# LIS-TU-Berlin/SVN-ICP

Measured on AMD Instinct MI355X. Metric: scan-pair registrations/sec at N particles x M source pts, 1/2/4/8 GPU, higher is better.
Workload: dtype f64; 1 GPU; C3: 128 particles SVN-ICP, 131072-pt source vs 262144-pt target, K=100, I=20, max_dist=1.0, lr=1.0, SVNFullGrad=False, correspondence=fast, early stop off; synthetic 64-beam scans (seed 20250718); particles=128, target_points=262144, knn_count=100, parallelism=single GPU

## Files before the change

### svn-icp_amd/csrc/knn_tiles.hip

```cpp
#include "kernels.hpp"
#include "stein_split_device.hpp"

namespace svnicp {

namespace {

constexpr int T = 8;
constexpr int STEP = kWave * T;
constexpr int QW = 64;
constexpr int WAVES = 4;
constexpr int QCAP = 1024;
constexpr int SL = 512;
constexpr int NSQ = 4;
constexpr int MAX_TILES = 8192;
constexpr int QB = 16;
constexpr double kU = 5.9604644775390625e-08;
constexpr float kEpsTile = 56.0f * 5.9604644775390625e-08f;

struct alignas(16) QF { float x, y, z, thr; };
struct alignas(16) QD { double x, y, z, tau; };

__device__ __forceinline__ void wave_sync() {
  __builtin_amdgcn_fence(__ATOMIC_ACQ_REL, "wavefront");
  __builtin_amdgcn_wave_barrier();
}
__device__ __forceinline__ bool ent_less(double da, int ia, double db, int ib) {
  return (da < db) || (da == db && ia < ib);
}
__device__ void bitonic_sort(double* sd, int* si, int S, int lane) {
  for (int k = 2; k <= S; k <<= 1)
    for (int j = k >> 1; j > 0; j >>= 1) {
      for (int e = lane; e < (S >> 1); e += kWave) {
        const int a = ((e & ~(j - 1)) << 1) | (e & (j - 1)), b = a | j;
        const bool up = (a & k) == 0;
        const double da = sd[a], db = sd[b];
        const int ia = si[a], ib = si[b];
        if (ent_less(db, ib, da, ia) == up) { sd[a] = db; si[a] = ib; sd[b] = da; si[b] = ia; }
      }
      wave_sync();
    }
}
__device__ void bitonic_sort128_f32(float* v, int lane) {
  for (int k = 2; k <= 128; k <<= 1)
    for (int j = k >> 1; j > 0; j >>= 1) {
      const int a = ((lane & ~(j - 1)) << 1) | (lane & (j - 1)), b = a | j;
      const bool up = (a & k) == 0;
      const float va = v[a], vb = v[b];
      if ((vb < va) == up) { v[a] = vb; v[b] = va; }
      wave_sync();
    }
}
__device__ __forceinline__ float next_down(float f) {
  if (f == 0.0f) return -1.401298464e-45f;
  int b = __float_as_int(f); b += (f > 0.0f) ? -1 : 1; return __int_as_float(b);
}
__device__ __forceinline__ float next_up(float f) {
  if (f == 0.0f) return 1.401298464e-45f;
  int b = __float_as_int(f); b += (f > 0.0f) ? 1 : -1; return __int_as_float(b);
}
__device__ __forceinline__ float f32_floor(double v) { float f = (float)v; return ((double)f > v) ? next_down(f) : f; }
__device__ __forceinline__ float f32_ceil(double v) { float f = (float)v; return ((double)f < v) ? next_up(f) : f; }
__device__ __forceinline__ float f32_round_up(double v) {
  float f = (float)v;
  if ((double)f < v) f = __int_as_float(__float_as_int(f) + 1);
  return f;
}
__device__ __forceinline__ float filter_threshold(double tau, double E) {
  if (!(tau < __builtin_huge_val())) return __builtin_huge_valf();
  const double r = sqrt(tau) * (1.0 + 1e-15) + 3.4641016151377553 * kU * E;
  return f32_round_up((r * r) * (1.0 + 5.0 * kU + 1e-6));
}
__device__ __forceinline__ float box_lb2(float alo0, float alo1, float alo2, float ahi0, float ahi1, float ahi2,
                                         float blo0, float blo1, float blo2, float bhi0, float bhi1, float bhi2) {
  const float g0 = __builtin_fmaxf(0.0f, __builtin_fmaxf(blo0 - ahi0, alo0 - bhi0));
  const float g1 = __builtin_fmaxf(0.0f, __builtin_fmaxf(blo1 - ahi1, alo1 - bhi1));
  const float g2 = __builtin_fmaxf(0.0f, __builtin_fmaxf(blo2 - ahi2, alo2 - bhi2));
  return (g0 * g0 + g1 * g1 + g2 * g2) * 0.999999f;
}

struct alignas(16) QRec { double x, y, z, tau; int cnt; int row; float thr, tb; };

__device__ __forceinline__ int pool_read(const KnnTilesArgs& a, int64_t r, int e) {
  if (e < kTilesBase) return a.pool[r * kTilesBase + e];
  const int o = e - kTilesBase;
  const int id = a.chunk_tab[r * kTilesChunks + (o / kTilesChunk)];
  return a.arena[(int64_t)id * kTilesChunk + (o % kTilesChunk)];
}

struct P3 { double x, y, z; };
__device__ __forceinline__ P3 target_row(const KnnTilesArgs& a, bool on, int i) {
  P3 c{0.0, 0.0, 0.0};
  if (on) { const double* p = a.tgt + 3 * (int64_t)i; c.x = p[0]; c.y = p[1]; c.z = p[2]; }
  return c;
}
__device__ __forceinline__ void write_table_row(const KnnTilesArgs& a, int64_t b, int r0, const P3 c0, int r1, const P3 c1, double* sd, int lane) {
  const int K = a.K;
  const bool on0 = r0 >= 0 && r0 < K, on1 = r1 >= 0 && r1 < K;
  const double x0 = c0.x, y0 = c0.y, z0 = c0.z, x1 = c1.x, y1 = c1.y, z1 = c1.z;
  float* rb = reinterpret_cast<float*>(sd);
  double* anc = sd + 256;
  wave_sync();
  if (on0 && r0 == 0) { anc[0] = x0; anc[1] = y0; anc[2] = z0; }
  if (on1 && r1 == 0) { anc[0] = x1; anc[1] = y1; anc[2] = z1; }
  wave_sync();
  const double a0 = anc[0], a1 = anc[1], a2 = anc[2];
  if (on0) *reinterpret_cast<float4*>(rb + 4 * r0) = table_row(x0, y0, z0, a0, a1, a2);
  if (on1) *reinterpret_cast<float4*>(rb + 4 * r1) = table_row(x1, y1, z1, a0, a1, a2);
  for (int k = K + lane; k < 128; k += kWave) *reinterpret_cast<float4*>(rb + 4 * k) = table_sentinel_row();
  wave_sync();
  float cm = 0.0f;
  for (int k = lane; k < K; k += kWave) cm = table_row_cmax(cm, *reinterpret_cast<const float4*>(rb + 4 * k));
  cm = table_cmax_wave(cm);
  if (lane == 0) {
    a.tbl_cmax[b] = cm;
    a.tbl_anchor[3 * b] = a0; a.tbl_anchor[3 * b + 1] = a1; a.tbl_anchor[3 * b + 2] = a2;
  }
  table_store_rows(rb, a.tbl_a, b, lane);
}

__device__ void select_query(const KnnTilesArgs& a, int64_t r, const QRec& rec, double* sd, int* si, int lane) {
  const int K = a.K, S2 = a.S2;
  const int64_t b = rec.row;
  const int n_first = rec.cnt;
  const double qx = rec.x, qy = rec.y, qz = rec.z;
  double tau = rec.tau;
  if (a.stat_n && lane == 0) a.stat_n[b] = n_first;
  const int n = n_first;
  bool ok = n <= S2;
  int m = 0;
  constexpr int NBR = 8;
  static_assert(NBR * kWave == kTilesBase, "the register path reads the query's own pool row only");
  if (ok && n <= NBR * kWave) {
    int slot[NBR], orig[NBR];
    double d[NBR];
#pragma unroll
    for (int j = 0; j < NBR; ++j) {
      const int e = j * kWave + lane;
      slot[j] = (j * kWave < n && e < n) ? a.pool[r * (int64_t)kTilesBase + e] : -1;
    }
#pragma unroll
    for (int j = 0; j < NBR; ++j) {
      d[j] = __builtin_huge_val(); orig[j] = 0;
      if (j * kWave < n && slot[j] >= 0) {
        orig[j] = a.torig[slot[j]];
        const double dx = qx - a.tx[slot[j]], dy = qy - a.ty[slot[j]], dz = qz - a.tz[slot[j]];
        d[j] = (dx * dx + dy * dy) + dz * dz;
      }
    }
    if (n > 2 * kWave && n >= K) {
      auto count_le = [&](double t) -> int {
        int c = 0;
#pragma unroll
        for (int j = 0; j < NBR; ++j)
          if (j * kWave < n) c += __popcll(__ballot(slot[j] >= 0 && d[j] <= t));
        return c;
      };
      double lo = 0.0, hi = tau;
      if (!(hi < __builtin_huge_val())) {
        double mx = 0.0;
#pragma unroll
        for (int j = 0; j < NBR; ++j) if (slot[j] >= 0) mx = fmax(mx, d[j]);
        for (int off = 32; off > 0; off >>= 1) mx = fmax(mx, __shfl_xor(mx, off, kWave));
        hi = mx;
      }
      const double target = 0.5 * (K + 2 * kWave);
      double t = hi * (double)__builtin_powf((float)(target / n), 0.6666667f);
      for (int it = 0; it < 48; ++it) {
        if (!(t > lo && t < hi)) t = 0.5 * (lo + hi);
        if (!(t > lo && t < hi)) break;
        const int c = count_le(t);
        if (c < K) lo = t;
        else { hi = t; if (c <= 2 * kWave) break; }
        t = 0.5 * (lo + hi);
      }
      tau = hi < tau ? hi : tau;
    }
#pragma unroll
    for (int j = 0; j < NBR; ++j) {
      if (j * kWave < n) {
        const bool pass = slot[j] >= 0 && d[j] <= tau;
        const unsigned long long pm = __ballot(pass);
        const int pos = m + (int)__builtin_amdgcn_mbcnt_hi((unsigned int)(pm >> 32), __builtin_amdgcn_mbcnt_lo((unsigned int)pm, 0u));
        if (pass && pos < SL) { sd[pos] = d[j]; si[pos] = orig[j]; }
        m += __popcll(pm);
      }
    }
    ok = m >= K && m <= SL;
  } else if (ok) {
    if (n > SL / 2) {
      double m1 = __builtin_huge_val(), m2 = __builtin_huge_val();
      for (int e = lane; e < n; e += kWave) {
        const int slot = pool_read(a, r, e);
        const double dx = qx - a.tx[slot], dy = qy - a.ty[slot], dz = qz - a.tz[slot];
        const double d = (dx * dx + dy * dy) + dz * dz;
        m2 = d < m1 ? m1 : (d < m2 ? d : m2);
        m1 = d < m1 ? d : m1;
      }
      sd[2 * lane] = m1; sd[2 * lane + 1] = m2; si[2 * lane] = 0; si[2 * lane + 1] = 0;
      wave_sync();
      bitonic_sort(sd, si, 128, lane);
      const double t2 = sd[K - 1];
      wave_sync();
      tau = t2 < tau ? t2 : tau;
    }
    for (int e0 = 0; e0 < n; e0 += kWave) {
      const int e = e0 + lane;
      bool pass = false;
      double d = 0.0;
      int orig = 0;
      if (e < n) {
        const int slot = pool_read(a, r, e);
        orig = a.torig[slot];
        const double dx = qx - a.tx[slot], dy = qy - a.ty[slot], dz = qz - a.tz[slot];
        d = (dx * dx + dy * dy) + dz * dz;
        pass = d <= tau;
      }
      const unsigned long long pm = __ballot(pass);
      const int pos = m + (int)__builtin_amdgcn_mbcnt_hi((unsigned int)(pm >> 32), __builtin_amdgcn_mbcnt_lo((unsigned int)pm, 0u));
      if (pass && pos < SL) { sd[pos] = d; si[pos] = orig; }
      m += __popcll(pm);
    }
    ok = m >= K && m <= SL;
  }
  if (!ok) {
    if (lane == 0) {
      const int slot = atomicAdd(a.fail_count, 1);
      a.fail_list[slot] = (int32_t)b;
      if (a.fail_tau) a.fail_tau[slot] = (n <= S2 && m < K) ? __builtin_huge_val() : tau;
    }
    wave_sync();
    return;
  }
  if (m <= 2 * kWave) {
    for (int e = m + lane; e < 2 * kWave + 8; e += kWave) { sd[e] = __builtin_huge_val(); si[e] = 0x7fffffff; }
    wave_sync();
    const int e0 = lane, e1 = lane + kWave;
    const double d0 = e0 < m ? sd[e0] : 0.0, d1 = e1 < m ? sd[e1] : 0.0;
    const int i0 = e0 < m ? si[e0] : 0, i1 = e1 < m ? si[e1] : 0;
    const P3 c0 = target_row(a, a.tbl_a && e0 < m, i0), c1 = target_row(a, a.tbl_a && e1 < m, i1);
    int* flag = si + 2 * kWave + 8;
    flag[lane] = 0; flag[lane + kWave] = 0;
    int r0 = 0, r1 = 0;
    for (int j0 = 0; j0 < m; j0 += 8) {
      double dj[8];
#pragma unroll
      for (int u = 0; u < 8; ++u) dj[u] = sd[j0 + u];
#pragma unroll
      for (int u = 0; u < 8; ++u) {
        r0 += dj[u] < d0 ? 1 : 0;
        r1 += dj[u] < d1 ? 1 : 0;
      }
    }
    wave_sync();
    if (e0 < m) atomicAdd(&flag[r0], 1);
    if (e1 < m) atomicAdd(&flag[r1], 1);
    wave_sync();
    if (__ballot((e0 < m && flag[r0] > 1) || (e1 < m && flag[r1] > 1))) {
      for (int j = 0; j < m; ++j) {
        const double dj = sd[j];
        const int ij = si[j];
        r0 += (dj == d0 && ij < i0) ? 1 : 0;
        r1 += (dj == d1 && ij < i1) ? 1 : 0;
      }
    }
    if (e0 < m && r0 < K) { a.out_idx[b * K + r0] = i0; if (a.out_d2) a.out_d2[b * K + r0] = d0; }
    if (e1 < m && r1 < K) { a.out_idx[b * K + r1] = i1; if (a.out_d2) a.out_d2[b * K + r1] = d1; }
    if (a.tbl_a) write_table_row(a, b, e0 < m ? r0 : -1, c0, e1 < m ? r1 : -1, c1, sd, lane);
    wave_sync();
  } else {
    int S = 256;
    while (S < m) S <<= 1;
    for (int e = m + lane; e < S; e += kWave) { sd[e] = __builtin_huge_val(); si[e] = 0x7fffffff; }
    wave_sync();
    bitonic_sort(sd, si, S, lane);
    for (int e = lane; e < K; e += kWave) { a.out_idx[b * K + e] = si[e]; if (a.out_d2) a.out_d2[b * K + e] = sd[e]; }
    if (a.tbl_a) {
      const int e1 = lane + kWave;
      write_table_row(a, b, lane, target_row(a, lane < K, si[lane]), e1, target_row(a, e1 < K, e1 < K ? si[e1] : 0), sd, lane);
    }
    wave_sync();
  }
}

__global__ __launch_bounds__(256) void k_knn_seed(KnnTilesArgs a) {
  extern __shared__ __align__(16) unsigned char smem[];
  const int lane = threadIdx.x & (kWave - 1);
  const int wave = __builtin_amdgcn_readfirstlane(threadIdx.x >> 6);
  const int K = a.K, n_tiles = a.n_tiles;
  constexpr size_t kShared = sizeof(QD) * QW + sizeof(QF) * QW + 4 * sizeof(int) * QW + sizeof(unsigned int) * (MAX_TILES / 32);
  constexpr size_t kScratch = sizeof(float2) * QB * kWave + 512;
  static_assert(QB * WAVES == QW, "one batch per wave");
  QD* qd = reinterpret_cast<QD*>(smem);
  QF* qf = reinterpret_cast<QF*>(smem + sizeof(QD) * QW);
  int* cnt = reinterpret_cast<int*>(smem + (sizeof(QD) + sizeof(QF)) * QW);
  int* qb = cnt + QW;
  float* thrb = reinterpret_cast<float*>(qb + QW);
  int* spare = reinterpret_cast<int*>(thrb + QW);
  unsigned int* tbits = reinterpret_cast<unsigned int*>(spare + QW);
  unsigned char* scratch = smem + kShared + kScratch * wave;
  float2* lm = reinterpret_cast<float2*>(scratch);

  const unsigned int grp = blockIdx.x;
  const int64_t q0 = a.b_lo + (int64_t)grp * QW;
  const int nq = (a.b_hi - q0) < QW ? (int)(a.b_hi - q0) : QW;
  const double Et = __longlong_as_double((long long)*a.emax_bits);

  unsigned long long tphase = a.phase_cycles ? __builtin_readcyclecounter() : 0ull;
  unsigned long long pacc[8] = {0, 0, 0, 0, 0, 0, 0, 0};
  auto phase_mark = [&](int i) {
    if (!a.phase_cycles) return;
    const unsigned long long now = __builtin_readcyclecounter();
    pacc[i] += now - tphase;
    tphase = now;
  };
  float wlo0 = 0.f, wlo1 = 0.f, wlo2 = 0.f, whi0 = 0.f, whi1 = 0.f, whi2 = 0.f;
  const int nwords = (n_tiles + 31) >> 5;
  if (wave == 0) {
    const bool act = lane < nq;
    const int64_t b = act ? (int64_t)a.qorder[q0 - a.b_lo + lane] : 0;
    QD s; s.x = s.y = s.z = 0.0; s.tau = 0.0;
    if (act) {
      stage_a_query(a.pose, a.src[3 * b], a.src[3 * b + 1], a.src[3 * b + 2], &s.x, &s.y, &s.z);
    }
    qd[lane] = s;
    QF f; f.x = (float)s.x; f.y = (float)s.y; f.z = (float)s.z; f.thr = -1.0f;
    qf[lane] = f;
    cnt[lane] = 0; qb[lane] = (int)b; thrb[lane] = -1.0f;
    const float inf = __builtin_huge_valf();
    wlo0 = act ? f32_floor(s.x) : inf; wlo1 = act ? f32_floor(s.y) : inf; wlo2 = act ? f32_floor(s.z) : inf;
    whi0 = act ? f32_ceil(s.x) : -inf; whi1 = act ? f32_ceil(s.y) : -inf; whi2 = act ? f32_ceil(s.z) : -inf;
    for (int off = 32; off > 0; off >>= 1) {
      wlo0 = __builtin_fminf(wlo0, __shfl_xor(wlo0, off, kWave)); whi0 = __builtin_fmaxf(whi0, __shfl_xor(whi0, off, kWave));
      wlo1 = __builtin_fminf(wlo1, __shfl_xor(wlo1, off, kWave)); whi1 = __builtin_fmaxf(whi1, __shfl_xor(whi1, off, kWave));
      wlo2 = __builtin_fminf(wlo2, __shfl_xor(wlo2, off, kWave)); whi2 = __builtin_fmaxf(whi2, __shfl_xor(whi2, off, kWave));
    }
  }
  wave_sync();
  const float* bx_lo0 = a.tile_box, *bx_lo1 = a.tile_box + n_tiles, *bx_lo2 = a.tile_box + 2 * (size_t)n_tiles;
  const float* bx_hi0 = a.tile_box + 3 * (size_t)n_tiles, *bx_hi1 = a.tile_box + 4 * (size_t)n_tiles,
             * bx_hi2 = a.tile_box + 5 * (size_t)n_tiles;

  {
    if (wave == 0) {
      for (int e = lane; e < nwords; e += kWave) tbits[e] = 0u;
      wave_sync();
      const float px = qf[lane].x, py = qf[lane].y, pz = qf[lane].z;
      unsigned long long best[NSQ];
#pragma unroll
      for (int i = 0; i < NSQ; ++i) best[i] = ~0ull;
      float4* boxs = reinterpret_cast<float4*>(scratch);
      const int n_groups = (n_tiles + kWave - 1) / kWave;
      unsigned int gkey[2] = {0xffffffffu, 0xffffffffu};
      for (int g = 0; g < n_groups; ++g) {
        const int tl = g * kWave + lane;
        const float inf = __builtin_huge_valf();
        float lo0 = inf, lo1 = inf, lo2 = inf, hi0 = -inf, hi1 = -inf, hi2 = -inf;
        if (tl < n_tiles) { lo0 = bx_lo0[tl]; lo1 = bx_lo1[tl]; lo2 = bx_lo2[tl]; hi0 = bx_hi0[tl]; hi1 = bx_hi1[tl]; hi2 = bx_hi2[tl]; }
        for (int off = 32; off > 0; off >>= 1) {
          lo0 = __builtin_fminf(lo0, __shfl_xor(lo0, off, kWave)); hi0 = __builtin_fmaxf(hi0, __shfl_xor(hi0, off, kWave));
          lo1 = __builtin_fminf(lo1, __shfl_xor(lo1, off, kWave)); hi1 = __builtin_fmaxf(hi1, __shfl_xor(hi1, off, kWave));
          lo2 = __builtin_fminf(lo2, __shfl_xor(lo2, off, kWave)); hi2 = __builtin_fmaxf(hi2, __shfl_xor(hi2, off, kWave));
        }
        const float glb = box_lb2(wlo0, wlo1, wlo2, whi0, whi1, whi2, lo0, lo1, lo2, hi0, hi1, hi2);
        const unsigned int key = (glb < inf) ? ((__float_as_uint(glb) & ~127u) | (unsigned int)g) : 0xffffffffu;
        if (lane == (g & (kWave - 1))) gkey[g >> 6] = key;
      }
      for (;;) {
        unsigned int kmin = gkey[0] < gkey[1] ? gkey[0] : gkey[1];
        for (int off = 32; off > 0; off >>= 1) { const unsigned int o = __shfl_xor(kmin, off, kWave); kmin = o < kmin ? o : kmin; }
        if (kmin == 0xffffffffu) break;
        float w4 = -__builtin_huge_valf();
        if (lane < nq) w4 = best[NSQ - 1] == ~0ull ? __builtin_huge_valf() : __uint_as_float((unsigned int)(best[NSQ - 1] >> 32));
        for (int off = 32; off > 0; off >>= 1) w4 = __builtin_fmaxf(w4, __shfl_xor(w4, off, kWave));
        if (__uint_as_float(kmin & ~127u) > w4) break;
        const int gsel = (int)(kmin & 127u);
        if (lane == (gsel & (kWave - 1))) gkey[gsel >> 6] = 0xffffffffu;
        const int t0 = gsel * kWave;
        const int tl = t0 + lane;
        if (tl < n_tiles) {
          boxs[2 * lane] = make_float4(bx_lo0[tl], bx_lo1[tl], bx_lo2[tl], bx_hi0[tl]);
          boxs[2 * lane + 1] = make_float4(bx_hi1[tl], bx_hi2[tl], 0.f, 0.f);
        }
        wave_sync();
        const int cntt = (n_tiles - t0) < kWave ? (n_tiles - t0) : kWave;
#pragma unroll 4
        for (int i = 0; i < cntt; ++i) {
          const float4 b0 = boxs[2 * i], b1 = boxs[2 * i + 1];
          const float l0 = b0.x, l1 = b0.y, l2 = b0.z, h0 = b0.w, h1 = b1.x, h2 = b1.y;
          const int tile = t0 + i;
          const float lb = box_lb2(px, py, pz, px, py, pz, l0, l1, l2, h0, h1, h2);
          const float c0 = px - 0.5f * (l0 + h0), c1 = py - 0.5f * (l1 + h1), c2 = pz - 0.5f * (l2 + h2);
          const float score = lb + 1e-3f * (c0 * c0 + c1 * c1 + c2 * c2);
          unsigned long long key = (score < __builtin_huge_valf()) ? (((unsigned long long)__float_as_uint(score) << 32) | (unsigned int)tile) : ~0ull;
#pragma unroll
          for (int u = 0; u < NSQ; ++u) {
            const unsigned long long lo = key < best[u] ? key : best[u];
            key = key < best[u] ? best[u] : key;
            best[u] = lo;
          }
        }
        wave_sync();
      }
      if (lane < nq) {
#pragma unroll
        for (int i = 0; i < NSQ; ++i)
          if (best[i] != ~0ull) { const unsigned int t = (unsigned int)(best[i] & 0xffffffffull); atomicOr(&tbits[t >> 5], 1u << (t & 31)); }
      }
    }
    phase_mark(0);
    __syncthreads();
    phase_mark(3);
    const int qb0 = wave * QB;
    if (qb0 < nq) {
      const int nb = (nq - qb0) < QB ? (nq - qb0) : QB;
      for (int e = lane; e < QB * kWave; e += kWave) lm[e] = make_float2(__builtin_huge_valf(), __builtin_huge_valf());
      wave_sync();
      for (int wd = 0; wd < nwords; ++wd) {
        unsigned int bits = __builtin_amdgcn_readfirstlane(tbits[wd]);
        while (bits) {
          const int tile = (wd << 5) + (int)__builtin_ctz(bits);
          bits &= bits - 1;
          if (a.phase_cycles) pacc[4] += 1;
          const int64_t tb = (int64_t)tile * STEP;
          float x[T], y[T], z[T];
#pragma unroll
          for (int t = 0; t < T; ++t) { x[t] = a.txf[tb + t * kWave + lane]; y[t] = a.tyf[tb + t * kWave + lane]; z[t] = a.tzf[tb + t * kWave + lane]; }
          for (int q = 0; q < nb; ++q) {
            const float4 cur = *reinterpret_cast<const float4*>(&qf[qb0 + q]);
            float2 m = lm[q * kWave + lane];
#pragma unroll
            for (int t = 0; t < T; ++t) {
              const float dx = cur.x - x[t], dy = cur.y - y[t], dz = cur.z - z[t];
              float d = __builtin_fmaf(dz, dz, __builtin_fmaf(dy, dy, dx * dx));
              d = __builtin_fminf(d, __builtin_huge_valf());
              m.y = __builtin_amdgcn_fmed3f(m.x, m.y, d);
              m.x = __builtin_fminf(m.x, d);
            }
            lm[q * kWave + lane] = m;
          }
        }
      }
      wave_sync();
      phase_mark(5);
      for (int q = 0; q < nb; ++q) {
        const float2 m = lm[q * kWave + lane];
        const unsigned int kx = __float_as_uint(m.x), ky = __float_as_uint(m.y);
        unsigned int kth = 0u;
        for (int bit = 30; bit >= 0; --bit) {
          const unsigned int t_try = kth | ((1u << bit) - 1u);
          const int c = __popcll(__ballot(kx <= t_try)) + __popcll(__ballot(ky <= t_try));
          if (c < K) kth |= 1u << bit;
        }
        if (lane == 0) spare[qb0 + q] = (int)kth;
      }
      phase_mark(6);
    }
    phase_mark(1);
    __syncthreads();
    phase_mark(3);
    if (wave == 0 && lane < nq) {
      const double tv = (double)__uint_as_float((unsigned int)spare[lane]);
      const double E = fmax(Et, fmax(fabs(qd[lane].x), fmax(fabs(qd[lane].y), fabs(qd[lane].z))));
      double tau = __builtin_huge_val();
      if (tv < (double)__builtin_huge_valf()) {
        const double r = sqrt(tv) * (1.0 + 1e-6) + 4.0 * kU * E;
        tau = (r * r) * (1.0 + 1e-12);
      }
      qd[lane].tau = tau;
      const float thr = filter_threshold(tau, E);
      qf[lane].thr = thr;
      float tb = __builtin_huge_valf();
      if (thr < __builtin_huge_valf()) {
        const double rb = sqrt((double)thr) + 2.0 * kU * E;
        tb = f32_round_up((rb * rb) * (1.0 + 1e-6));
      }
      thrb[lane] = tb;
    }
    wave_sync();
  }

  if (wave == 0 && lane < nq) {
    QRec rec;
    rec.x = qd[lane].x; rec.y = qd[lane].y; rec.z = qd[lane].z; rec.tau = qd[lane].tau;
    rec.cnt = 0; rec.row = qb[lane]; rec.thr = qf[lane].thr; rec.tb = thrb[lane];
    reinterpret_cast<QRec*>(a.qrec)[q0 + lane] = rec;
  }
  phase_mark(1);
  if (a.phase_cycles && lane == 0) {
#pragma unroll
    for (int i = 0; i < 5; ++i) atomicAdd(&a.phase_cycles[i], pacc[i]);
    unsigned long long* pw = a.phase_cycles + 8 + 8 * ((size_t)grp * WAVES + wave);
#pragma unroll
    for (int i = 0; i < 7; ++i) pw[i] = pacc[i];
  }
}

template <int SW, bool MF>
__global__ __launch_bounds__(64 * SW) __attribute__((amdgpu_waves_per_eu(4, 4))) void k_knn_scan_tiles(KnnTilesArgs a) {
  __shared__ __align__(16) QF s_qf[QW];
  __shared__ int s_cnt[QW];
  __shared__ int s_ticket;
  __shared__ __align__(16) int2 s_queue[SW][QCAP];
  __shared__ __align__(16) float4 s_lb[MF ? SW : 1][QW];
  __shared__ float s_lth[MF ? SW : 1][QW];
  __shared__ int s_lq[MF ? SW : 1][QW];
  const int lane = threadIdx.x & (kWave - 1);
  const int wave = __builtin_amdgcn_readfirstlane(threadIdx.x >> 6);
  const int S2 = a.S2, n_tiles = a.n_tiles;
  int2* queue = s_queue[wave];
  const unsigned int ngrp = gridDim.x;
  const unsigned int grp = (unsigned int)(((unsigned long long)blockIdx.x * a.group_stride) % ngrp);
  const int64_t q0 = a.b_lo + (int64_t)grp * QW;
  const int nq = (a.b_hi - q0) < QW ? (int)(a.b_hi - q0) : QW;
  QRec* recs = reinterpret_cast<QRec*>(a.qrec);
  unsigned long long tphase = a.phase_cycles ? __builtin_readcyclecounter() : 0ull;
  unsigned long long pacc[8] = {0, 0, 0, 0, 0, 0, 0, 0};
  auto phase_mark = [&](int i) {
    if (!a.phase_cycles) return;
    const unsigned long long now = __builtin_readcyclecounter();
    pacc[i] += now - tphase;
    tphase = now;
  };
  float gx = 0.f, gy = 0.f, gz = 0.f, gtb = -1.0f, gthr = -1.0f;
  float wlo0, wlo1, wlo2, whi0, whi1, whi2, tmax;
  {
    const bool act = lane < nq;
    QF f; f.x = f.y = f.z = 0.f; f.thr = -1.0f;
    const float inf = __builtin_huge_valf();
    wlo0 = wlo1 = wlo2 = inf; whi0 = whi1 = whi2 = -inf;
    if (act) {
      const QRec rec = recs[q0 + lane];
      f.x = (float)rec.x; f.y = (float)rec.y; f.z = (float)rec.z; f.thr = rec.thr;
      gtb = rec.tb; gthr = rec.thr;
      wlo0 = f32_floor(rec.x); wlo1 = f32_floor(rec.y); wlo2 = f32_floor(rec.z);
      whi0 = f32_ceil(rec.x); whi1 = f32_ceil(rec.y); whi2 = f32_ceil(rec.z);
    }
    gx = f.x; gy = f.y; gz = f.z;
    if (wave == 0) { s_qf[lane] = f; s_cnt[lane] = 0; }
    if (threadIdx.x == 0) s_ticket = 0;
    tmax = gtb;
    for (int off = 32; off > 0; off >>= 1) {
      wlo0 = __builtin_fminf(wlo0, __shfl_xor(wlo0, off, kWave)); whi0 = __builtin_fmaxf(whi0, __shfl_xor(whi0, off, kWave));
      wlo1 = __builtin_fminf(wlo1, __shfl_xor(wlo1, off, kWave)); whi1 = __builtin_fmaxf(whi1, __shfl_xor(whi1, off, kWave));
      wlo2 = __builtin_fminf(wlo2, __shfl_xor(wlo2, off, kWave)); whi2 = __builtin_fmaxf(whi2, __shfl_xor(whi2, off, kWave));
      tmax = __builtin_fmaxf(tmax, __shfl_xor(tmax, off, kWave));
    }
  }
  __syncthreads();
  const float* bx_lo0 = a.tile_box, *bx_lo1 = a.tile_box + n_tiles, *bx_lo2 = a.tile_box + 2 * (size_t)n_tiles;
  const float* bx_hi0 = a.tile_box + 3 * (size_t)n_tiles, *bx_hi1 = a.tile_box + 4 * (size_t)n_tiles,
             * bx_hi2 = a.tile_box + 5 * (size_t)n_tiles;
  int qcount = 0;
  auto put = [&](int q, int pos, bool on, int slot) {
    const int64_t r = q0 + q;
    if (on && pos < kTilesBase) a.pool[r * kTilesBase + pos] = slot;
    const bool ovf = on && pos >= kTilesBase && pos < S2;
    if (__ballot(ovf)) {
      const int o = pos - kTilesBase;
      int32_t* tab = a.chunk_tab + r * kTilesChunks + (ovf ? o / kTilesChunk : 0);
      if (ovf && (o % kTilesChunk) == 0) {
        int id = atomicAdd(a.chunk_tab + a.tab_rows * (int64_t)kTilesChunks, 1) + 1;
        if (id >= a.arena_cap) id = -2;
        __hip_atomic_store(tab, id, __ATOMIC_RELAXED, __HIP_MEMORY_SCOPE_AGENT);
      }
      if (ovf) {
        int id = -1;
        for (int spin = 0; spin < (1 << 22) && id == -1; ++spin) {
          id = __hip_atomic_load(tab, __ATOMIC_RELAXED, __HIP_MEMORY_SCOPE_AGENT);
          if (id == -1) __builtin_amdgcn_s_sleep(2);
        }
        if (id >= 0) a.arena[(int64_t)id * kTilesChunk + (o % kTilesChunk)] = slot;
        else atomicMax(&s_cnt[q], 1 << 24);
      }
    }
  };
  auto flush = [&]() {
    wave_sync();
    for (int e0 = 0; e0 < qcount; e0 += kWave) {
      const int e = e0 + lane;
      const bool on = e < qcount;
      const int2 ent = on ? queue[e] : make_int2(0, -1 - lane);
      const int prev = __shfl_up(ent.y, 1, kWave);
      const unsigned long long lead = __ballot(on && (lane == 0 || ent.y != prev));
      const unsigned long long upto = lead & (~0ull >> (63 - lane));
      const int L = 63 - (int)__builtin_clzll(upto | 1ull);
      const unsigned long long after = lead & ~((2ull << L) - 1ull);
      const int nvalid = (qcount - e0) < kWave ? (qcount - e0) : kWave;
      const int end = after ? (int)__builtin_ctzll(after) : nvalid;
      const int q = ent.y & (QW - 1);
      int base = 0;
      if (on && lane == L) base = atomicAdd(&s_cnt[q], end - L);
      base = __shfl(base, L, kWave);
      put(q, base + (lane - L), on, ent.x);
    }
    qcount = 0;
    wave_sync();
  };
  auto flush_quads = [&]() {
    wave_sync();
    for (int e0 = 0; e0 < qcount; e0 += kWave) {
      const int e = e0 + lane;
      const bool on = e < qcount;
      const int2 ent = on ? queue[e] : make_int2(0, 0);
      const int q = ent.y & (QW - 1);
      const unsigned int bits = ((unsigned int)ent.y >> 8) & 15u;
      const int n = __popc(bits);
      int pos = 0;
      if (n) pos = atomicAdd(&s_cnt[q], n);
      const int64_t r = q0 + q;
      const bool ovf = n > 0 && pos + n > kTilesBase && pos < S2;
      const bool any_ovf = __ballot(ovf) != 0ull;
      if (ovf) {
#pragma unroll
        for (int j = 0; j < 4; ++j) {
          const int o = pos + j - kTilesBase;
          if (j < n && o >= 0 && pos + j < S2 && (o % kTilesChunk) == 0) {
            int id = atomicAdd(a.chunk_tab + a.tab_rows * (int64_t)kTilesChunks, 1) + 1;
            if (id >= a.arena_cap) id = -2;
            __hip_atomic_store(a.chunk_tab + r * kTilesChunks + o / kTilesChunk, id, __ATOMIC_RELAXED, __HIP_MEMORY_SCOPE_AGENT);
          }
        }
      }
#pragma unroll
      for (int i = 0; i < 4; ++i) {
        const bool hit = (bits >> i) & 1u;
        if (hit && pos < kTilesBase) a.pool[r * kTilesBase + pos] = ent.x + i;
        if (any_ovf && hit && pos >= kTilesBase && pos < S2) {
          const int o = pos - kTilesBase;
          int32_t* tab = a.chunk_tab + r * kTilesChunks + o / kTilesChunk;
          int id = -1;
          for (int spin = 0; spin < (1 << 22) && id == -1; ++spin) {
            id = __hip_atomic_load(tab, __ATOMIC_RELAXED, __HIP_MEMORY_SCOPE_AGENT);
            if (id == -1) __builtin_amdgcn_s_sleep(2);
          }
          if (id >= 0) a.arena[(int64_t)id * kTilesChunk + (o % kTilesChunk)] = ent.x + i;
          else atomicMax(&s_cnt[q], 1 << 24);
        }
        pos += hit ? 1 : 0;
      }
    }
    qcount = 0;
    wave_sync();
  };
  {
    auto next_ticket = [&]() { int v = 0; if (lane == 0) v = atomicAdd(&s_ticket, 1); return __builtin_amdgcn_readfirstlane(v); };
    int my = next_ticket(), seen = 0;
    for (int t0 = 0; t0 < n_tiles; t0 += kWave) {
      const int tl = t0 + lane;
      bool need = false;
      if (tl < n_tiles)
        need = box_lb2(wlo0, wlo1, wlo2, whi0, whi1, whi2, bx_lo0[tl], bx_lo1[tl], bx_lo2[tl], bx_hi0[tl], bx_hi1[tl], bx_hi2[tl]) <= tmax;
      const unsigned long long any = __ballot(need);
      const int n_here = __popcll(any);
      while (my < seen + n_here) {
        unsigned long long rem = any;
        for (int k = my - seen; k > 0; --k) rem &= rem - 1;
        const int tile = t0 + (int)__builtin_ctzll(rem);
        my = next_ticket();
        if (a.phase_cycles) pacc[5] += 1;
        const float l0 = bx_lo0[tile], l1 = bx_lo1[tile], l2 = bx_lo2[tile], h0 = bx_hi0[tile], h1 = bx_hi1[tile], h2 = bx_hi2[tile];
        unsigned long long qmask = __ballot(lane < nq && box_lb2(gx, gy, gz, gx, gy, gz, l0, l1, l2, h0, h1, h2) <= gtb);
        if (!qmask) continue;
        if (a.phase_cycles) pacc[6] += __popcll(qmask);
        const int64_t tb = (int64_t)tile * STEP;
        if constexpr (MF) {
          const int mj = lane & 15, mk = lane >> 4;
          const float4* rowp = a.tile_a + (size_t)tile * STEP + lane;
          v4f ra = *reinterpret_cast<const v4f*>(rowp), rb_ = *reinterpret_cast<const v4f*>(rowp + kWave);
          const float4 org = a.tile_o[tile];
          const int nlive = __popcll(qmask), nbat = (nlive + 15) >> 4;
          {
            const float x0 = gx - org.x, x1 = gy - org.y, x2 = gz - org.z;
            const float X2 = __builtin_fmaf(x2, x2, __builtin_fmaf(x1, x1, x0 * x0));
            const float Xn = __builtin_amdgcn_sqrtf(X2) * 1.000002f;
            const float eps = __builtin_fmaf(kEpsTile * org.w, __builtin_fmaf(2.0f, Xn, org.w),
                                             __builtin_fmaf(12.0f * (float)kU, X2, __builtin_fmaf(4.0f * (float)kU, gthr, 1e-30f * (1.0f + Xn + org.w))));
            float th = (gthr - X2) + eps;
            th = th < __builtin_huge_valf() ? th : __builtin_huge_valf();
            const bool live = (qmask >> lane) & 1ull;
            const int pos = (int)__builtin_amdgcn_mbcnt_hi((unsigned int)(qmask >> 32), __builtin_amdgcn_mbcnt_lo((unsigned int)qmask, 0u));
            if (live) { s_lb[wave][pos] = make_float4(-2.0f * x0, -2.0f * x1, -2.0f * x2, 1.0f); s_lth[wave][pos] = th; s_lq[wave][pos] = lane; }
            const int padi = nlive + lane;
            if (padi < 16 * nbat) { s_lb[wave][padi] = make_float4(0.f, 0.f, 0.f, 0.f); s_lth[wave][padi] = -__builtin_huge_valf(); s_lq[wave][padi] = 0; }
          }
          wave_sync();
#pragma nounroll
          for (int c = 0; c < 4; ++c) {
            bf8 afr[8];
#pragma unroll
            for (int k = 0; k < 4; ++k) { afr[k] = split_a3(ra[k]); afr[4 + k] = split_a3(rb_[k]); }
            if (c < 3) { ra = *reinterpret_cast<const v4f*>(rowp + (2 * c + 2) * kWave); rb_ = *reinterpret_cast<const v4f*>(rowp + (2 * c + 3) * kWave); }
#pragma nounroll
            for (int b = 0; b < nbat; ++b) {
              const int col = 16 * b + mj;
              const float bv = reinterpret_cast<const float*>(&s_lb[wave][col])[mk];
              const float th = s_lth[wave][col];
              const bool valid = col < nlive;
              const unsigned long long vmask = __ballot(valid);
              const bf8 bfr = split_b3(bv);
              const v4f zero = {0.0f, 0.0f, 0.0f, 0.0f};
              const int q = s_lq[wave][col];
              const int srow = __builtin_amdgcn_readfirstlane((int)tb + 128 * c);
              v4f dcur = __builtin_amdgcn_mfma_f32_16x16x32_bf16(afr[0], bfr, zero, 0, 0, 0);
              v4f dnext = __builtin_amdgcn_mfma_f32_16x16x32_bf16(afr[1], bfr, zero, 0, 0, 0);
#pragma unroll
              for (int k = 0; k < 8; ++k) {
                v4f dn2 = dnext;
                if (k + 2 < 8) dn2 = __builtin_amdgcn_mfma_f32_16x16x32_bf16(afr[k + 2 < 8 ? k + 2 : 0], bfr, zero, 0, 0, 0);
                const v4f dk = dcur;
                dcur = dnext; dnext = dn2;
                const float m4 = fmin_raw(fmin3_raw(dk[0], dk[1], dk[2]), dk[3]);
                const bool any4 = !(m4 > th);
                const unsigned long long m = __ballot(any4) & vmask;
                if (m) {
                  const unsigned int bits = (!(dk[0] > th) ? 0x100u : 0u) | (!(dk[1] > th) ? 0x200u : 0u) |
                                            (!(dk[2] > th) ? 0x400u : 0u) | (!(dk[3] > th) ? 0x800u : 0u);
                  const int pos = qcount + (int)__builtin_amdgcn_mbcnt_hi((unsigned int)(m >> 32), __builtin_amdgcn_mbcnt_lo((unsigned int)m, 0u));
                  if (any4 && valid) queue[pos] = make_int2(srow + 16 * k + 4 * mk, q | (int)bits);
                  qcount += __popcll(m);
                }
              }
              qcount = __builtin_amdgcn_readfirstlane(qcount);
              if (qcount > QCAP - 8 * kWave) flush_quads();
            }
          }
          wave_sync();
          continue;
        }
        float x[T], y[T], z[T];
#pragma unroll
        for (int t = 0; t < T; ++t) { x[t] = a.txf[tb + t * kWave + lane]; y[t] = a.tyf[tb + t * kWave + lane]; z[t] = a.tzf[tb + t * kWave + lane]; }
        while (qmask) {
          const int q = (int)__builtin_ctzll(qmask);
          qmask &= qmask - 1;
          const float4 cur = *reinterpret_cast<const float4*>(&s_qf[q]);
          float d[T];
#pragma unroll
          for (int t = 0; t < T; ++t) {
            const float dx = cur.x - x[t], dy = cur.y - y[t], dz = cur.z - z[t];
            d[t] = __builtin_fmaf(dz, dz, __builtin_fmaf(dy, dy, dx * dx));
          }
          float dm = __builtin_fminf(__builtin_fminf(d[0], d[1]), d[2]);
#pragma unroll
          for (int t = 3; t + 1 < T; t += 2) dm = __builtin_fminf(__builtin_fminf(dm, d[t]), d[t + 1]);
          if constexpr ((T - 3) % 2 == 1) dm = __builtin_fminf(dm, d[T - 1]);
          if (__ballot(dm <= cur.w)) {
#pragma unroll
            for (int t = 0; t < T; ++t) {
              const bool hit = d[t] <= cur.w;
              const unsigned long long m = __ballot(hit);
              if (m) {
                const int pos = qcount + (int)__builtin_amdgcn_mbcnt_hi((unsigned int)(m >> 32), __builtin_amdgcn_mbcnt_lo((unsigned int)m, 0u));
                if (hit) queue[pos] = make_int2((int)(tb + t * kWave + lane), q);
                qcount += __popcll(m);
              }
            }
            qcount = __builtin_amdgcn_readfirstlane(qcount);
            if (qcount > QCAP - STEP) flush();
          }
        }
      }
      seen += n_here;
    }
    if constexpr (MF) flush_quads(); else flush();
  }
  phase_mark(2);
  __syncthreads();
  phase_mark(3);
  if (wave == 0 && lane < nq) recs[q0 + lane].cnt = s_cnt[lane];
  if (a.phase_cycles && lane == 0) {
    atomicAdd(&a.phase_cycles[2], pacc[2]); atomicAdd(&a.phase_cycles[3], pacc[3]);
    atomicAdd(&a.phase_cycles[5], pacc[5]); atomicAdd(&a.phase_cycles[6], pacc[6]);
    atomicMax(&a.phase_cycles[7], pacc[2]);
  }
}

__global__ __launch_bounds__(256) void k_knn_select(KnnTilesArgs a) {
  __shared__ __align__(16) double s_sd[WAVES][SL];
  __shared__ int s_si[WAVES][SL];
  const int lane = threadIdx.x & (kWave - 1);
  const int wave = __builtin_amdgcn_readfirstlane(threadIdx.x >> 6);
  const QRec* recs = reinterpret_cast<const QRec*>(a.qrec);
  for (int64_t r = a.b_lo + (int64_t)blockIdx.x * WAVES + wave; r < a.b_hi; r += (int64_t)gridDim.x * WAVES) {
    const QRec rec = recs[r];
    select_query(a, r, rec, s_sd[wave], s_si[wave], lane);
  }
}

__global__ __launch_bounds__(256) void k_candidate_dist2(const double* __restrict__ src, Pose0 pose, const double* __restrict__ tgt, int64_t M,
                                                         const int32_t* __restrict__ idx, int64_t B, int K, double* __restrict__ d2) {
  const int lane = threadIdx.x & (kWave - 1);
  const int wave = __builtin_amdgcn_readfirstlane(threadIdx.x >> 6);
  for (int64_t b = (int64_t)blockIdx.x * WAVES + wave; b < B; b += (int64_t)gridDim.x * WAVES) {
    double qx, qy, qz;
    stage_a_query(pose, src[3 * b], src[3 * b + 1], src[3 * b + 2], &qx, &qy, &qz);
    int first0 = 0x7fffffff;
    for (int k0 = 0; k0 < K && first0 == 0x7fffffff; k0 += kWave) {
      const unsigned long long z = __ballot(k0 + lane < K && idx[b * K + k0 + lane] == 0);
      if (z) first0 = k0 + (int)__builtin_ctzll(z);
    }
    for (int k = lane; k < K; k += kWave) {
      int64_t i = idx[b * K + k];
      const bool pad = i == 0 && k > first0;
      i = i < 0 ? 0 : (i >= M ? M - 1 : i);
      const double dx = qx - tgt[3 * i], dy = qy - tgt[3 * i + 1], dz = qz - tgt[3 * i + 2];
      const double d = (dx * dx + dy * dy) + dz * dz;
      d2[b * K + k] = (pad || d != d) ? 0.0 : d;
    }
  }
}

}

hipError_t launch_candidate_dist2(const double* src, const Pose0& pose, const double* tgt, int64_t M, const int32_t* idx, int64_t B, int K,
                                  double* d2, hipStream_t st) {
  if (B <= 0 || K <= 0) return hipSuccess;
  int64_t nb = (B + WAVES - 1) / WAVES;
  if (nb > 65536) nb = 65536;
  hipLaunchKernelGGL(k_candidate_dist2, dim3((unsigned)nb), dim3(256), 0, st, src, pose, tgt, M, idx, B, K, d2);
  return hipGetLastError();
}

static_assert(STEP == kTileSlots && MAX_TILES == kMaxTiles, "knn_tiles_applicable (stage_a_plan.hpp) speaks of this kernel's tiles");

hipError_t launch_knn_tiles(const KnnTilesArgs& a, hipStream_t st) {
  const int64_t nq = a.b_hi - a.b_lo;
  if (nq <= 0) return hipSuccess;
  const int64_t nb = (nq + QW - 1) / QW;
  if (a.n_tiles > MAX_TILES) return hipErrorInvalidValue;
  const size_t smem = sizeof(QD) * QW + sizeof(QF) * QW + 4 * sizeof(int) * QW + sizeof(unsigned int) * (MAX_TILES / 32) +
                      (sizeof(float2) * QB * kWave + 512) * WAVES;
  hipError_t e = hipFuncSetAttribute(reinterpret_cast<const void*>(k_knn_seed),
                                     hipFuncAttributeMaxDynamicSharedMemorySize, (int)smem);
  if (e != hipSuccess) return e;
  hipLaunchKernelGGL(k_knn_seed, dim3((unsigned)nb), dim3(256), smem, st, a);
  e = hipGetLastError();
  if (e != hipSuccess) return e;
  const dim3 sgrid((unsigned)((nq + QW - 1) / QW));
  if (a.prefilter_mfma) {
    if (a.scan_split == 4) hipLaunchKernelGGL((k_knn_scan_tiles<4, true>), sgrid, dim3(256), 0, st, a);
    else hipLaunchKernelGGL((k_knn_scan_tiles<8, true>), sgrid, dim3(512), 0, st, a);
  } else {
    if (a.scan_split == 4) hipLaunchKernelGGL((k_knn_scan_tiles<4, false>), sgrid, dim3(256), 0, st, a);
    else hipLaunchKernelGGL((k_knn_scan_tiles<8, false>), sgrid, dim3(512), 0, st, a);
  }
  e = hipGetLastError();
  if (e != hipSuccess) return e;
  int64_t nbs = (nq + WAVES - 1) / WAVES;
  if (nbs > 65536) nbs = 65536;
  hipLaunchKernelGGL(k_knn_select, dim3((unsigned)nbs), dim3(256), 0, st, a);
  return hipGetLastError();
}

}
```

Baseline: 150.2 registrations/s.

## Replace all-pairs rank counting with bucketed counting sort in kNN select

```diff
diff --git a/svn-icp_amd/csrc/knn_select_rank.hpp b/svn-icp_amd/csrc/knn_select_rank.hpp
--- /dev/null
+++ b/svn-icp_amd/csrc/knn_select_rank.hpp
@@ -0,0 +1,24 @@
+#pragma once
+
+#if defined(__HIPCC__)
+#define SVNICP_RANK_FN __device__ __forceinline__
+#else
+#define SVNICP_RANK_FN inline
+#endif
+
+namespace svnicp {
+
+constexpr int kRankBuckets = 256;
+
+SVNICP_RANK_FN double rank_scale(double top) {
+  if (!(top > 0.0) || !(top < __builtin_huge_val())) return 0.0;
+  const double s = (double)kRankBuckets / top;
+  return s < __builtin_huge_val() ? s : 1.7976931348623157e308;
+}
+
+SVNICP_RANK_FN int rank_bucket(double d, double scale) {
+  const double v = d * scale;
+  return v < (double)(kRankBuckets - 1) ? (int)v : kRankBuckets - 1;
+}
+
+}
diff --git a/svn-icp_amd/csrc/knn_tiles.hip b/svn-icp_amd/csrc/knn_tiles.hip
--- a/svn-icp_amd/csrc/knn_tiles.hip
+++ b/svn-icp_amd/csrc/knn_tiles.hip
@@ -1,4 +1,5 @@
 #include "kernels.hpp"
+#include "knn_select_rank.hpp"
 #include "stein_split_device.hpp"
 
 namespace svnicp {
@@ -26,6 +27,15 @@
 }
 __device__ __forceinline__ bool ent_less(double da, int ia, double db, int ib) {
   return (da < db) || (da == db && ia < ib);
+}
+__device__ __forceinline__ int wave_inclusive_scan(int v, int lane) {
+  v += __builtin_amdgcn_update_dpp(0, v, 0x111, 0xf, 0xf, false);
+  v += __builtin_amdgcn_update_dpp(0, v, 0x112, 0xf, 0xf, false);
+  v += __builtin_amdgcn_update_dpp(0, v, 0x114, 0xf, 0xf, false);
+  v += __builtin_amdgcn_update_dpp(0, v, 0x118, 0xf, 0xf, false);
+  const int t0 = __builtin_amdgcn_readlane(v, 15), t1 = __builtin_amdgcn_readlane(v, 31), t2 = __builtin_amdgcn_readlane(v, 47);
+  const int row = lane >> 4;
+  return v + (row > 0 ? t0 : 0) + (row > 1 ? t1 : 0) + (row > 2 ? t2 : 0);
 }
 __device__ void bitonic_sort(double* sd, int* si, int S, int lane) {
   for (int k = 2; k <= S; k <<= 1)
@@ -232,35 +242,63 @@
     return;
   }
   if (m <= 2 * kWave) {
-    for (int e = m + lane; e < 2 * kWave + 8; e += kWave) { sd[e] = __builtin_huge_val(); si[e] = 0x7fffffff; }
     wave_sync();
     const int e0 = lane, e1 = lane + kWave;
-    const double d0 = e0 < m ? sd[e0] : 0.0, d1 = e1 < m ? sd[e1] : 0.0;
-    const int i0 = e0 < m ? si[e0] : 0, i1 = e1 < m ? si[e1] : 0;
-    const P3 c0 = target_row(a, a.tbl_a && e0 < m, i0), c1 = target_row(a, a.tbl_a && e1 < m, i1);
-    int* flag = si + 2 * kWave + 8;
-    flag[lane] = 0; flag[lane + kWave] = 0;
-    int r0 = 0, r1 = 0;
-    for (int j0 = 0; j0 < m; j0 += 8) {
-      double dj[8];
-#pragma unroll
-      for (int u = 0; u < 8; ++u) dj[u] = sd[j0 + u];
-#pragma unroll
-      for (int u = 0; u < 8; ++u) {
-        r0 += dj[u] < d0 ? 1 : 0;
-        r1 += dj[u] < d1 ? 1 : 0;
-      }
-    }
-    wave_sync();
-    if (e0 < m) atomicAdd(&flag[r0], 1);
-    if (e1 < m) atomicAdd(&flag[r1], 1);
-    wave_sync();
-    if (__ballot((e0 < m && flag[r0] > 1) || (e1 < m && flag[r1] > 1))) {
-      for (int j = 0; j < m; ++j) {
-        const double dj = sd[j];
-        const int ij = si[j];
-        r0 += (dj == d0 && ij < i0) ? 1 : 0;
-        r1 += (dj == d1 && ij < i1) ? 1 : 0;
+    const bool on0 = e0 < m, on1 = e1 < m;
+    const double d0 = on0 ? sd[e0] : __builtin_huge_val(), d1 = on1 ? sd[e1] : __builtin_huge_val();
+    const int i0 = on0 ? si[e0] : 0x7fffffff, i1 = on1 ? si[e1] : 0x7fffffff;
+    const P3 c0 = target_row(a, a.tbl_a && on0, i0), c1 = target_row(a, a.tbl_a && on1, i1);
+    int* cnt = si + 4 * kWave;
+    reinterpret_cast<int4*>(cnt)[lane] = make_int4(0, 0, 0, 0);
+    double top = tau;
+    if (!(top < __builtin_huge_val())) {
+      top = fmax(on0 ? d0 : 0.0, on1 ? d1 : 0.0);
+      for (int off = 32; off > 0; off >>= 1) top = fmax(top, __shfl_xor(top, off, kWave));
+    }
+    const double scale = rank_scale(top);
+    const int k0 = rank_bucket(d0, scale), k1 = rank_bucket(d1, scale);
+    wave_sync();
+    const int o0 = on0 ? atomicAdd(&cnt[k0], 1) : 0, o1 = on1 ? atomicAdd(&cnt[k1], 1) : 0;
+    wave_sync();
+    {
+      const int4 c = reinterpret_cast<const int4*>(cnt)[lane];
+      const int s = (c.x + c.y) + (c.z + c.w);
+      int st = wave_inclusive_scan(s, lane) - s;
+      int4 p;
+      p.x = st | (c.x << 8); st += c.x;
+      p.y = st | (c.y << 8); st += c.y;
+      p.z = st | (c.z << 8); st += c.z;
+      p.w = st | (c.w << 8);
+      reinterpret_cast<int4*>(cnt)[lane] = p;
+    }
+    wave_sync();
+    const int p0 = on0 ? cnt[k0] : 0, p1 = on1 ? cnt[k1] : 0;
+    const int s0 = p0 & 0xff, n0 = p0 >> 8, s1 = p1 & 0xff, n1 = p1 >> 8;
+    if (on0) { sd[s0 + o0] = d0; si[s0 + o0] = i0; } else { sd[e0] = d0; si[e0] = i0; }
+    if (on1) { sd[s1 + o1] = d1; si[s1 + o1] = i1; } else { sd[e1] = d1; si[e1] = i1; }
+    if (lane == 0) { sd[2 * kWave] = __builtin_huge_val(); si[2 * kWave] = 0x7fffffff; }
+    wave_sync();
+    const int nmax = n0 > n1 ? n0 : n1;
+    int r0 = s0, r1 = s1, q0 = 0, q1 = 0;
+    for (int t = 0; __ballot(t < nmax); t += 2) {
+      double x0[2], x1[2];
+#pragma unroll
+      for (int u = 0; u < 2; ++u) {
+        const int a0 = s0 + t + u, a1 = s1 + t + u;
+        x0[u] = sd[a0 < 2 * kWave ? a0 : 2 * kWave];
+        x1[u] = sd[a1 < 2 * kWave ? a1 : 2 * kWave];
+      }
+#pragma unroll
+      for (int u = 0; u < 2; ++u) {
+        r0 += x0[u] < d0 ? 1 : 0; q0 += x0[u] == d0 ? 1 : 0;
+        r1 += x1[u] < d1 ? 1 : 0; q1 += x1[u] == d1 ? 1 : 0;
+      }
+    }
+    if (__ballot(q0 > 1 || q1 > 1)) {
+      for (int t = 0; __ballot(t < nmax); ++t) {
+        const int a0 = s0 + (t < n0 ? t : 0), a1 = s1 + (t < n1 ? t : 0);
+        r0 += (t < n0 && sd[a0] == d0 && si[a0] < i0) ? 1 : 0;
+        r1 += (t < n1 && sd[a1] == d1 && si[a1] < i1) ? 1 : 0;
       }
     }
     if (e0 < m && r0 < K) { a.out_idx[b * K + r0] = i0; if (a.out_d2) a.out_d2[b * K + r0] = d0; }
@@ -777,7 +815,7 @@
 
 __global__ __launch_bounds__(256) void k_knn_select(KnnTilesArgs a) {
   __shared__ __align__(16) double s_sd[WAVES][SL];
-  __shared__ int s_si[WAVES][SL];
+  __shared__ __align__(16) int s_si[WAVES][SL];
   const int lane = threadIdx.x & (kWave - 1);
   const int wave = __builtin_amdgcn_readfirstlane(threadIdx.x >> 6);
   const QRec* recs = reinterpret_cast<const QRec*>(a.qrec);
```

Measured after the change: 150.6 registrations/s, median of 4. No clear change (+0.3%).
